# ScottHCL/recommend

Hardware: AMD Instinct MI355X
Metric: ranked samples/sec (fwd+bwd) at B=4096 seq=128; AUC parity vs ref (higher is better)
Workload: dtype f32-emulated (fp16-pair / split-bf16); 1 GPU; C2: OneTrans 4L d128 H4 f512 L_NS12 L_S128 (seq 3x42), Criteo-shape 13 dense + 26 ids, replicated tables, fwd+bwd+optimizer; global_batch=4096, per_gpu_batch=4096, seq_len=128, parallelism=dp1

## Files before the change

### include/onetrans_hip.h

```cpp
#ifndef ONETRANS_HIP_H
#define ONETRANS_HIP_H

#include <stddef.h>
#include <stdint.h>

#ifdef __cplusplus
extern "C" {
#endif

#define OT_OK 0
#define OT_ERR_INVALID_ARG 1
#define OT_ERR_UNSUPPORTED 2
#define OT_ERR_HIP 3

#define OT_GEMM_NN 0
#define OT_GEMM_NT 1

#define OT_AX_NONE 0
#define OT_AX_RMSNORM 1
#define OT_AX_GELU 2
#define OT_AX_BF16 4
#define OT_AX_BF16_RMSNORM 5

#define OT_EPI_BIAS 1
// ... 99 lines not shown
int ot_mixed_gemm_rms_img(int mode, const float* A, int64_t lda, int K, const int32_t* in_rows,
                          int a_xform, const float* a_rstd, const float* a_gamma,
                          const float* W, int64_t w_gstride, int64_t ldw, int N,
                          const int32_t* tile_group, int ntiles,
                          const float* bias, int64_t bias_gstride,
                          float* C, int64_t ldc, const int32_t* out_rows, int epi,
                          const float* res, int64_t ldres, int res_tok,
                          const float* aux, int64_t ldaux,
                          uint32_t seed, uint32_t site, float drop_rate, int tail_K, int tail_I,
                          const int32_t* tail_pos, const ot_rms_epilogue* rms, const uint16_t* b_image,
                          int image_ntn, int image_tn0, int precision, void* stream);

typedef struct ot_ffn_fused_args {
  size_t struct_size;
  const float* x1; int64_t ldx1;
  const int32_t* rows;
  const int32_t* tile_group; int ntiles;
  const float* rstd;
  const uint16_t* w1_image; int w1_groups;
  const uint16_t* w2_image; int w2_groups;
  const float* b1; int64_t b1_gstride;
  const float* b2; int64_t b2_gstride;
  int f;
  float* u_out; int64_t ldu;
  float* u_amax;
  float* x2; int64_t ldx2;
  float* rstd_out; float eps;
  uint32_t seed, site; float drop_rate;
  int tail_K, tail_I; const int32_t* tail_pos;
} ot_ffn_fused_args;
int ot_ffn_fused_fwd(const ot_ffn_fused_args* args, void* stream);
int ot_ffn_fused(int on);

int ot_attn_fwd(const float* qkv, int64_t ld, int B, int H, int I, int K, const int32_t* qpos,
                int head_dim, float* out, float* lse, int precision, void* stream);
size_t ot_attn_fwd_fp8_workspace_size(int B, int H, int I, int head_dim);
int ot_attn_fwd_fp8(const float* qkv, int64_t ld, int B, int H, int I, int K, const int32_t* qpos,
                    int head_dim, float* out, float* lse, void* workspace, size_t ws_bytes, void* stream);
#define OT_FP8_DEQUANT 1
#define OT_FP8_TWO_TERM 2
int ot_attn_fwd_fp8_ex(float* qkv, int64_t ld, int B, int H, int I, int K, const int32_t* qpos, int head_dim,
                       float* out, float* lse, void* workspace, size_t ws_bytes, int flags, void* stream);
int ot_attn_fwd_fp8_deq16(const float* qkv, int64_t ld, int B, int H, int I, int K, const int32_t* qpos,
                          int head_dim, float* out, float* lse, void* workspace, size_t ws_bytes, int flags,
                          uint16_t* deq16, void* stream);
size_t ot_attn_bwd_workspace_size(int B, int H, int K);
int ot_attn_bwd(const float* qkv, int64_t ld, const float* out, const float* dout, const float* lse,
                int B, int H, int I, int K, const int32_t* qpos, int head_dim, float* dqkv, float* delta_ws,
                int precision, void* stream);
size_t ot_attn_bwd_ex_workspace_size(int B, int H, int I, int K, int head_dim, int selected, int precision);
int ot_attn_bwd_ex(const float* qkv, int64_t ld, const float* out, const float* dout, const float* lse,
                   int B, int H, int I, int K, const int32_t* qpos, int head_dim, float* dqkv, void* workspace,
                   size_t ws_bytes, int precision, void* stream);
#define OT_ATTN_DQKV_BF16 1
#define OT_ATTN_QKV_BF16 2
#define OT_ATTN_DQ_PART_BF16 4
int ot_attn_bwd_dqkv_bf16_supported(int I, int K, int head_dim, int selected, int precision);
int ot_attn_bwd_bf16_forms(int I, int K, int head_dim, int selected, int precision);
size_t ot_attn_bwd_flags_workspace_size(int B, int H, int I, int K, int head_dim, int selected, int flags, int precision);
int ot_attn_slice_supported(int I, int K, int head_dim, int selected);
int ot_attn_bwd_flags(const float* qkv, int64_t ld, const float* out, const float* dout, const float* lse,
                      int B, int H, int I, int K, const int32_t* qpos, int head_dim, void* dqkv, int flags,
                      void* workspace, size_t ws_bytes, int precision, void* stream);
int ot_attn_amax_supported(int I, int K, int head_dim, int selected, int precision);
int ot_attn_fwd_amax(const float* qkv, int64_t ld, int B, int H, int I, int K, const int32_t* qpos,
                     int head_dim, float* out, float* lse, float* amax, float* rowmax, int precision, void* stream);
// ... 211 lines not shown
```

### recommend_amd/_lib.py

```python

from __future__ import annotations

import ctypes
import os
from ctypes import c_float, c_int, c_int64, c_size_t, c_uint32, c_void_p, c_char_p

_HERE = os.path.dirname(os.path.abspath(__file__))
LIB_PATH = os.environ.get('ONETRANS_HIP_LIB') or os.path.join(_HERE, 'libonetrans_hip.so')
HEADER = os.path.join(os.path.dirname(_HERE), 'include', 'onetrans_hip.h')

OT_GEMM_NN, OT_GEMM_NT = 0, 1
OT_AX_NONE, OT_AX_RMSNORM, OT_AX_GELU, OT_AX_BF16, OT_AX_BF16_RMSNORM = 0, 1, 2, 4, 5
OT_EPI_BIAS, OT_EPI_GELU_BWD, OT_EPI_GELU = 1, 2, 4
OT_EPI_DROPOUT, OT_EPI_RESIDUAL, OT_EPI_ACCUMULATE = 8, 16, 32
OT_EPI_ROW_RSTD, OT_EPI_RMSNORM_BWD, OT_EPI_ROWDOT = 64, 128, 256
OT_EPI_C_BF16 = 512
OT_EPI_AUX_BF16 = 1024
OT_ATTN_DQKV_BF16 = 1
OT_ATTN_QKV_BF16 = 2
OT_ATTN_DQ_PART_BF16 = 4
OT_WG_D_BF16 = 8
OT_MATMUL_F32, OT_MATMUL_SPLIT_BF16, OT_MATMUL_BF16 = 0, 1, 2
OT_FP8_DEQUANT, OT_FP8_TWO_TERM = 1, 2
OT_RANK_SUM, OT_RANK_PRODUCT = 0, 1
RANK_MODES = {'sum': OT_RANK_SUM, 'product': OT_RANK_PRODUCT}
RANK_MAX_K = 1024
MATMUL_MODES = {'f32': OT_MATMUL_F32, 'split': OT_MATMUL_SPLIT_BF16, 'bf16': OT_MATMUL_BF16}


class RmsEpilogue(ctypes.Structure):
    _fields_ = [('struct_size', c_size_t), ('rstd_out', c_void_p), ('eps', c_float),
                ('x', c_void_p), ('ldx', c_int64), ('gamma', c_void_p), ('rstd', c_void_p),
                ('dres', c_void_p), ('lddres', c_int64), ('dres_tail_K', c_int), ('dres_tail_I', c_int),
                ('dres_tail_inv', c_void_p),
                ('dx_masked', c_void_p), ('lddxm', c_int64),
                ('dgamma', c_void_p), ('accumulate_dgamma', c_int),
                ('workspace', c_void_p), ('ws_bytes', c_size_t),
                ('rowdot', c_void_p), ('rowdot_n', c_int),
                ('gelu_out', c_void_p), ('ldgelu', c_int64),
                ('xn_out', c_void_p), ('ldxn', c_int64),
                ('c16_out', c_void_p), ('ldc16', c_int64),
                ('rowmax_out', c_void_p), ('rowmax_n', c_int),
                ('a_rowmax', c_void_p), ('a_rowmax_n', c_int),
                ('amax_out', c_void_p), ('rowabs_out', c_void_p), ('rowabs_n', c_int)]

class FfnFusedArgs(ctypes.Structure):
    _fields_ = [('struct_size', c_size_t), ('x1', c_void_p), ('ldx1', c_int64), ('rows', c_void_p),
                ('tile_group', c_void_p), ('ntiles', c_int), ('rstd', c_void_p),
                ('w1_image', c_void_p), ('w1_groups', c_int), ('w2_image', c_void_p), ('w2_groups', c_int),
                ('b1', c_void_p), ('b1_gstride', c_int64), ('b2', c_void_p), ('b2_gstride', c_int64),
                ('f', c_int), ('u_out', c_void_p), ('ldu', c_int64), ('u_amax', c_void_p),
                ('x2', c_void_p), ('ldx2', c_int64), ('rstd_out', c_void_p), ('eps', c_float),
                ('seed', c_uint32), ('site', c_uint32), ('drop_rate', c_float),
                ('tail_K', c_int), ('tail_I', c_int), ('tail_pos', c_void_p)]


class SeqTime(ctypes.Structure):
    _fields_ = [('times', c_void_p), ('stride_b', c_int64), ('L', ctypes.c_int32), ('map_off', ctypes.c_int32)]


class NsBag(ctypes.Structure):
    _fields_ = [('table', c_void_p), ('ids', c_void_p), ('weights', c_void_p), ('row_offset', c_int64),
                ('num_rows', c_int64), ('ids_stride', c_int64), ('weights_stride', c_int64),
                ('width', ctypes.c_int32), ('cap', ctypes.c_int32), ('col', ctypes.c_int32),
                ('pooling', ctypes.c_int32)]


OT_BAG_SUM, OT_BAG_MEAN = 0, 1
BAG_POOLINGS = {'sum': OT_BAG_SUM, 'mean': OT_BAG_MEAN}
NS_BAG_MAX = 32
NS_BAG_MAX_WIDTH = 256
SEQ_TIME_MAX_L = 4096
SEQ_TIME_MAX_SEQ = 32

P = c_void_p
I64 = c_int64

SIGNATURES = {
    'ot_version': (c_int, []),
    'ot_get_last_error_string': (c_char_p, []),
    'ot_gemm_tile_rows': (c_int, []),
    'ot_mixed_gemm': (c_int, [c_int, P, I64, c_int, P, c_int, P, P, P, I64, I64, c_int, P, c_int, P, I64,
                              P, I64, P, c_int, P, I64, c_int, P, I64, c_uint32, c_uint32, c_float, c_int,
                              c_int, P, c_int, P]),
    'ot_mixed_gemm_rms_workspace_size': (c_size_t, [c_int, c_int]),
    'ot_mixed_gemm_rms': (c_int, [c_int, P, I64, c_int, P, c_int, P, P, P, I64, I64, c_int, P, c_int, P, I64,
                                  P, I64, P, c_int, P, I64, c_int, P, I64, c_uint32, c_uint32, c_float, c_int,
                                  c_int, P, P, c_int, P]),
    'ot_wgrad_workspace_size': (c_size_t, [c_int, c_int, c_int]),
    'ot_mixed_gemm_wgrad': (c_int, [P, I64, P, c_int, P, P, P, I64, P, c_int, c_int, P, c_int, P, c_int, P,
                                    I64, P, I64, c_int, P, c_size_t, c_int, P]),
    'ot_mixed_gemm_wgrad_ex': (c_int, [P, I64, P, c_int, P, P, P, I64, P, c_int, c_int, P, c_int, P, c_int, P,
                                       I64, P, I64, c_int, P, c_size_t, P, P, c_int, P]),
    'ot_transpose_banks': (c_int, [P, P, P, c_int, I64, P]),
    'ot_mixed_gemm_img': (c_int, [c_int, P, I64, c_int, P, c_int, P, P, P, I64, I64, c_int, P, c_int, P, I64,
                                  P, I64, P, c_int, P, I64, c_int, P, I64, c_uint32, c_uint32, c_float, c_int,
                                  c_int, P, P, c_int, c_int, c_int, P]),
    'ot_mixed_gemm_rms_img': (c_int, [c_int, P, I64, c_int, P, c_int, P, P, P, I64, I64, c_int, P, c_int, P, I64,
                                      P, I64, P, c_int, P, I64, c_int, P, I64, c_uint32, c_uint32, c_float, c_int,
                                      c_int, P, P, P, c_int, c_int, c_int, P]),
    'ot_split_image_elems': (c_size_t, [c_int, c_int, c_int]),
    'ot_plane_wide': (c_int, [c_int]),
    'ot_wgrad_wide': (c_int, [c_int]),
    'ot_plane_rowmeta': (c_int, [c_int]),
    'ot_plane_panel': (c_int, [c_int]),
    'ot_plane_panel_launches': (c_int, []),
    'ot_ffn_fused_fwd': (c_int, [P, P]),
    'ot_ffn_fused': (c_int, [c_int]),
    'ot_split_images': (c_int, [P, P, c_int, I64, P, c_int, P]),
    'ot_attn_fwd': (c_int, [P, I64, c_int, c_int, c_int, c_int, P, c_int, P, P, c_int, P]),
    'ot_attn_fwd_fp8_workspace_size': (c_size_t, [c_int, c_int, c_int, c_int]),
    'ot_attn_fwd_fp8': (c_int, [P, I64, c_int, c_int, c_int, c_int, P, c_int, P, P, P, c_size_t, P]),
    'ot_attn_fwd_fp8_ex': (c_int, [P, I64, c_int, c_int, c_int, c_int, P, c_int, P, P, P, c_size_t, c_int, P]),
    'ot_attn_fwd_fp8_deq16': (c_int, [P, I64, c_int, c_int, c_int, c_int, P, c_int, P, P, P, c_size_t, c_int, P, P]),
    'ot_attn_bwd_workspace_size': (c_size_t, [c_int, c_int, c_int]),
    'ot_attn_bwd': (c_int, [P, I64, P, P, P, c_int, c_int, c_int, c_int, P, c_int, P, P, c_int, P]),
    'ot_attn_bwd_ex_workspace_size': (c_size_t, [c_int, c_int, c_int, c_int, c_int, c_int, c_int]),
    'ot_attn_bwd_ex': (c_int, [P, I64, P, P, P, c_int, c_int, c_int, c_int, P, c_int, P, P, c_size_t, c_int, P]),
    'ot_attn_bwd_dqkv_bf16_supported': (c_int, [c_int, c_int, c_int, c_int, c_int]),
    'ot_attn_bwd_bf16_forms': (c_int, [c_int, c_int, c_int, c_int, c_int]),
    'ot_attn_slice_supported': (c_int, [c_int, c_int, c_int, c_int]),
    'ot_attn_bwd_flags_workspace_size': (c_size_t, [c_int, c_int, c_int, c_int, c_int, c_int, c_int, c_int]),
    'ot_attn_bwd_flags': (c_int, [P, I64, P, P, P, c_int, c_int, c_int, c_int, P, c_int, P, c_int, P, c_size_t, c_int, P]),
    'ot_attn_fwd_cached': (c_int, [P, I64, P, I64, P, c_int, c_int, c_int, c_int, c_int, c_int, P, P]),
    'ot_attn_fwd_cached_lse': (c_int, [P, I64, P, I64, P, c_int, c_int, c_int, c_int, c_int, c_int, P, P, P]),
    'ot_attn_bwd_cached_workspace_size': (c_size_t, [c_int, c_int, c_int, c_int, c_int, c_int, c_int]),
    'ot_attn_bwd_cached': (c_int, [P, I64, P, I64, P, c_int, c_int, c_int, c_int, c_int, c_int, c_int, P, P, P, P, P,
                                   c_int, P, c_size_t, P]),
    'ot_attn_amax_supported': (c_int, [c_int, c_int, c_int, c_int, c_int]),
    'ot_attn_fwd_amax': (c_int, [P, I64, c_int, c_int, c_int, c_int, P, c_int, P, P, P, P, c_int, P]),
    'ot_attn_bwd_amax': (c_int, [P, I64, P, P, P, c_int, c_int, c_int, c_int, P, c_int, P, P, c_size_t, P, P, c_int,
                                 P]),
    'ot_pyramid_select': (c_int, [P, c_float, c_int, c_int, c_int, c_int, P, P, P, c_int, P]),
    'ot_rmsnorm_fwd': (c_int, [P, I64, P, P, I64, P, I64, c_int, c_float, P]),
    'ot_rmsnorm_bwd_workspace_size': (c_size_t, [I64, c_int]),
    'ot_rmsnorm_bwd': (c_int, [P, I64, P, I64, P, P, P, I64, c_int, c_int, P, P, I64, P, I64, c_uint32,
                               c_uint32, c_float, c_int, c_int, P, P, c_int, I64, c_int, P, c_size_t, P]),
    'ot_dropout_apply': (c_int, [P, I64, P, I64, I64, c_int, c_uint32, c_uint32, c_float, c_int, c_int, P, P]),
    'ot_dropout_apply_bf16': (c_int, [P, I64, P, I64, I64, c_int, c_uint32, c_uint32, c_float, c_int, c_int, P, P]),
    'ot_rows_absmax': (c_int, [P, I64, I64, c_int, P, c_int, P]),
    'ot_dropout_rowmax_supported': (c_int, [c_int]),
# ... 115 lines not shown
```

### recommend_amd/csrc/gemm_ffn.hip

```cpp
#include <atomic>
#include <cstdlib>
#include <mutex>

#include "gemm.h"

namespace ot {

#ifndef OT_FFN_NSTG
#define OT_FFN_NSTG 3
#endif
constexpr int FF_NST = OT_FFN_NSTG;
static_assert(FF_NST == 2 || FF_NST == 3, "fused FFN stage buffers");
constexpr int PG_A_BYTES = GT * 16 * 4;
constexpr int FF_STG = PG_A_BYTES + 2 * GT * 16 * 2;
constexpr int FF_TR_LD = 36;
constexpr int FF_TR_WAVE = 32 * FF_TR_LD * 4;
constexpr int FF_TR_OFF = FF_NST * FF_STG;
constexpr int FF_META_OFF = FF_TR_OFF + 4 * FF_TR_WAVE;
constexpr int FF_TAB_OFF = FF_META_OFF + GT * 4;
constexpr int FF_MAX_F = 1024;
static_assert(FF_META_OFF >= (64 * (GT + 4) + 8 * GT) * 4, "fused FFN: the epilogue tile overlays the row metadata");
static_assert(FF_TAB_OFF + (2 * FF_MAX_F + GT) * 4 <= 80 * 1024, "fused FFN LDS");
constexpr int ffn_lds(int f) { return FF_TAB_OFF + (2 * f + GT) * 4; }

// ... 210 lines not shown
          }
#pragma unroll
        for (int nb = 0; nb < 4; ++nb) acc2[nb] = mfma_pair_t(fw[nb], fh, acc2[nb]);
      }
    };
    stage2(0, acc1[0]);
    stage2(1, acc1[1]);
    stage2(2, acc1[2]);
    stage2(3, acc1[3]);
  }
#pragma unroll
  for (int nb = 0; nb < 4; ++nb)
#pragma unroll
    for (int qd = 0; qd < 4; ++qd) {
      const f32x4 cs = *reinterpret_cast<const f32x4*>(tab + 2 * q.f + 32 * nb + 8 * qd + 4 * h);
#pragma unroll
      for (int i = 0; i < 4; ++i) acc2[nb][4 * qd + i] *= hinv * cs[i];
    }
  asm volatile("s_waitcnt vmcnt(0) lgkmcnt(0)" ::: "memory");
  __syncthreads();
  gemm_vec_epilogue<EPIT, 5, false, 8, false>(p, acc2, smem, tm, 0, g, 0, -1, rmeta);
  if (q.u_amax) amax_flush(q.u_amax, am);
}

#ifndef OT_FFN_FUSED
#define OT_FFN_FUSED 1
#endif
static int ffn_fused_initial() {
  const char* e = getenv("ONETRANS_FFN_FUSED");
  return e && *e ? (atoi(e) != 0) : OT_FFN_FUSED;
}
static std::atomic<int> g_ffn_fused{ffn_fused_initial()};

}

using namespace ot;

extern "C" int ot_ffn_fused(int on) {
  const int old = g_ffn_fused.load(std::memory_order_relaxed);
  if (on >= 0) g_ffn_fused.store(on ? 1 : 0, std::memory_order_relaxed);
  return old;
}

extern "C" int ot_ffn_fused_fwd(const ot_ffn_fused_args* a, void* stream) {
  OT_REQUIRE(a, "ot_ffn_fused_fwd: null arguments");
  OT_REQUIRE(a->struct_size == sizeof(ot_ffn_fused_args),
             "ot_ffn_fused_fwd: ot_ffn_fused_args.struct_size %zu != %zu (header of another ot_version)",
             a->struct_size, sizeof(ot_ffn_fused_args));
  OT_REQUIRE(a->x1 && a->x2 && a->rstd && a->w1_image && a->w2_image && a->b1 && a->b2,
             "ot_ffn_fused_fwd: null operand");
  OT_REQUIRE(a->ntiles >= 0 && a->f >= GT && a->f % GT == 0 && a->f <= FF_MAX_F,
             "ot_ffn_fused_fwd: bad sizes ntiles=%d f=%d (f a multiple of %d up to %d)", a->ntiles, a->f, GT, FF_MAX_F);
  auto a16 = [](const void* q) { return ((uintptr_t)q & 15) == 0; };
  OT_REQUIRE(a->ldx1 >= GT && a->ldx2 >= GT && a->ldx1 % 4 == 0 && a->ldx2 % 4 == 0 && a16(a->x1) && a16(a->x2) &&
                 a16(a->b1) && a16(a->b2) && a->b1_gstride % 4 == 0 && a->b2_gstride % 4 == 0 && a16(a->w1_image) &&
                 a16(a->w2_image),
             "ot_ffn_fused_fwd: rows of %d floats, leading dimensions and bias strides multiples of 4, 16-B aligned "
             "operands", GT);
  OT_REQUIRE(!a->u_out || (a->ldu >= a->f && a->ldu % 4 == 0 && a16(a->u_out)),
             "ot_ffn_fused_fwd: u_out needs ldu >= f, ldu %% 4 == 0 and 16-B alignment");
  OT_REQUIRE(a->w1_groups >= 1 && a->w2_groups >= 1, "ot_ffn_fused_fwd: image group counts must be >= 1");
  OT_REQUIRE(a->w1_groups == 1 && a->w2_groups == 1 ? true : a->tile_group != nullptr,
             "ot_ffn_fused_fwd: grouped weight images need tile_group");
  OT_REQUIRE(a->drop_rate >= 0.f && a->drop_rate < 1.f, "ot_ffn_fused_fwd: drop_rate out of range");
  OT_REQUIRE(a->drop_rate == 0.f || (a->tail_K > 0 && a->tail_I >= a->tail_K), "ot_ffn_fused_fwd: bad tail map");
  if (a->ntiles == 0) return OT_OK;
  FfnArgs q{};
  GemmArgs& p = q.e;
  p.A = a->x1; p.lda = a->ldx1; p.K = GT; p.in_rows = a->rows; p.a_xform = OT_AX_RMSNORM; p.a_rstd = a->rstd;
// ... 43 lines not shown
```

### recommend_amd/kernels.py

```python

from __future__ import annotations

import contextlib
import ctypes
import functools
import os
import threading
from typing import Optional, Tuple, Union

import torch

from . import _lib
from ._lib import call, size

Ptrish = Union[None, torch.Tensor, Tuple[torch.Tensor, int]]


class Probe:

    def __init__(self):
        self.recs = []

    def begin(self):
        ev = torch.cuda.Event(enable_timing=True)
# ... 277 lines not shown
    return _lib.size('ot_plane_panel', int(on))


def plane_panel_launches() -> int:
    return _lib.size('ot_plane_panel_launches')


def ffn_fused(on: int = -1) -> int:
    return _lib.size('ot_ffn_fused', int(on))


FFN_FUSED_MAX_F = 1024


def ffn_fused_fwd(x1: Ptrish, ldx1: int, rows: Ptrish, tile_group: Ptrish, ntiles: int, rstd: Ptrish, w1_image,
                  w1_groups: int, w2_image, w2_groups: int, b1: Ptrish, b1_gstride: int, b2: Ptrish, b2_gstride: int,
                  f: int, x2: Ptrish, ldx2: int, *, u_out: Ptrish = None, ldu: int = 0, u_amax: Ptrish = None,
                  rstd_out: Ptrish = None, eps: float = 1e-6, seed: int = 0, site: int = 0, drop: float = 0.0,
                  tail: Tuple[int, int] = (1, 1), m_rows: int = 0) -> None:
    a = _lib.FfnFusedArgs(ctypes.sizeof(_lib.FfnFusedArgs), ptr(x1), ldx1, ptr(rows), ptr(tile_group), ntiles,
                          ptr(rstd), ptr(w1_image), int(w1_groups), ptr(w2_image), int(w2_groups), ptr(b1),
                          b1_gstride, ptr(b2), b2_gstride, f, ptr(u_out), ldu, ptr(u_amax), ptr(x2), ldx2,
                          ptr(rstd_out), float(eps), seed & 0xFFFFFFFF, site, float(drop), tail[0], tail[1],
                          _sel(tail))
    ev = _probe.begin() if _probe is not None else None
    call('ot_ffn_fused_fwd', ctypes.byref(a), stream())
    if ev is not None:
        M = m_rows or ntiles * 128
        _probe.end('mixed_gemm', 2.0 * M * 128 * f * 2, ev, f'ffn_fused M{M} f{f} u{int(u_out is not None)}',
                   4.0 * M * 128 * 3 + 4.0 * M * f * (u_out is not None)
                   + 4.0 * M * (1 + (rstd_out is not None)), 3)


def split_images(base, desc_dev, ndesc, total_units, img) -> None:
    call('ot_split_images', ptr(base), ptr(desc_dev), ndesc, total_units, ptr(img), _prec(), stream())


def attn_fwd(qkv: torch.Tensor, ld: int, B: int, H: int, I: int, K: int, hd: int, out: torch.Tensor,
             lse: torch.Tensor, qpos: Optional[torch.Tensor] = None, fp8: bool = False,
             dequant: bool = False, fp8_terms: int = 1, deq16: Optional[torch.Tensor] = None,
             amax: Optional[torch.Tensor] = None, rowmax: Optional[torch.Tensor] = None) -> None:
    if fp8 and fp8_terms not in (1, 2):
        raise ValueError(f'fp8_terms {fp8_terms}: 1 or 2')
    ws = None
    if fp8:
        ws = workspace(size('ot_attn_fwd_fp8_workspace_size', B, H, I, hd), qkv.device)
    ev = _probe.begin() if _probe is not None else None
    if fp8 and deq16 is not None:
        call('ot_attn_fwd_fp8_deq16', ptr(qkv), ld, B, H, I, K, ptr(qpos), hd, ptr(out), ptr(lse), ptr(ws),
             ws.numel(), _lib.OT_FP8_TWO_TERM if fp8_terms == 2 else 0, ptr(deq16), stream())
    elif fp8:
        call('ot_attn_fwd_fp8_ex', ptr(qkv), ld, B, H, I, K, ptr(qpos), hd, ptr(out), ptr(lse), ptr(ws),
             ws.numel(), (_lib.OT_FP8_DEQUANT if dequant else 0) | (_lib.OT_FP8_TWO_TERM if fp8_terms == 2 else 0),
             stream())
    elif amax is not None or rowmax is not None:
        call('ot_attn_fwd_amax', ptr(qkv), ld, B, H, I, K, ptr(qpos), hd, ptr(out), ptr(lse), ptr(amax), ptr(rowmax),
             _prec(), stream())
    else:
        call('ot_attn_fwd', ptr(qkv), ld, B, H, I, K, ptr(qpos), hd, ptr(out), ptr(lse), _prec(), stream())
    if ev is not None:
        _probe.end('attention', 4.0 * (K * I - K * (K - 1) / 2) * hd * H * B, ev,
                   f'fwd{"_fp8" if fp8 else ""} I{I} K{K} hd{hd}')


def attn_bwd_bf16_forms(I, K, hd, qpos=None) -> int:
    return int(_lib.load().ot_attn_bwd_bf16_forms(I, K, hd, int(qpos is not None), _prec()))
# ... 477 lines not shown
```

### recommend_amd/model.py

```python

from __future__ import annotations

import json
import os
from typing import Dict, List, Optional, Tuple

import numpy as np
import torch
import torch.nn as nn

from . import _lib
from . import kernels as K
from ._lib import (OT_AX_BF16, OT_AX_BF16_RMSNORM, OT_AX_GELU, OT_AX_RMSNORM, OT_EPI_ACCUMULATE, OT_EPI_AUX_BF16, OT_EPI_BIAS,
                   OT_EPI_C_BF16, OT_EPI_DROPOUT, OT_EPI_GELU_BWD, OT_EPI_RESIDUAL, OT_EPI_RMSNORM_BWD,
                   OT_EPI_ROW_RSTD, OT_EPI_ROWDOT, OT_GEMM_NN, OT_GEMM_NT, OT_WG_D_BF16, NS_FIELD_BYTES)
from .config import (OneTransConfig, check_bag_features, check_padding_mask, check_pyramid_select, check_seq_fusion,
                     get_model_config)
from .layout import TILE, FlatLayout, RowMap, build_map, head_map, identity_map, layer_maps, round_up
from .params import init_params, ns_table_offsets

RMS_EPS = 1e-6


class _Tokenize(torch.autograd.Function):
# ... 369 lines not shown
        nca, nct = maps['all'].chunks.shape[0], maps['tail'].chunks.shape[0]
        G = cfg.num_groups
        dx2 = dx2.contiguous()
        rowdot = None
        fused2 = m.fuse_bwd2 and not m.fuse_bwd and f % TILE == 0
        du_bf = (fused2 and h is not None and m.bimg(f'blk.{l}.w1', 'dgrad') is not None)
        out = (lambda name: bounds.out(l, name)) if bounds is not None else (lambda name: None)
        b_o, b_u = (bounds.get(l, 'o'), bounds.get(l, 'u')) if bounds is not None else (None, None)
        keep = (bounds.t,) if bounds is not None else ()
        pw2, pw1, pwo = (m.dgrad_pair(f'blk.{l}.{w}') for w in ('w2', 'w1', 'wo'))
        dy2_rep = rate > 0 and not du_bf
        b_dy2 = out('dy2') if dy2_rep else None
        rm_dy2 = (torch.empty(B * Kq, (d + 255) // 256, device=dev)
                  if dy2_rep and pw2 and K.dropout_rowmax_supported(d) else None)
        dy2 = dx2
        if rate > 0:
            dy2 = torch.empty(B * Kq, d, device=dev, dtype=torch.int16 if du_bf else torch.float32)
            K.dropout_apply(dx2, d, dy2, d, B * Kq, d, seed, 2 * l + 1, rate, tail, amax=b_dy2, rowmax=rm_dy2)
        pa2 = a_row_bounds(pw2, dy2, d, B * Kq, d, rm_dy2)
        dy_bf = dy2.dtype == torch.int16
        du = torch.empty(B * Kq, f, device=dev, dtype=torch.int16 if du_bf else torch.float32)
        cbf = OT_EPI_C_BF16 if du_bf else 0
        hbf = (torch.empty(B * Kq, f, dtype=torch.int16, device=dev)
               if h is None and fused2 and K.matmul_mode() == 'bf16' else None)
        if hbf is None:
            with m.side(u if h is None else h, dy2, *keep):
                K.wgrad(u if h is None else h, f, mt['rows'][1], dy2, d, mt['rows'][1], f, d, mt, nct, G,
                        m.g(f'blk.{l}.w2'), f * d, m.g(f'blk.{l}.b2'), d,
                        a_xform=(OT_AX_GELU if h is None else OT_AX_BF16) | (OT_WG_D_BF16 if dy_bf else 0),
                        accumulate=acc, device=dev, m_rows=maps['tail'].nrows, rowmap=maps['tail'],
                        a_bound=b_u if h is None else None, d_bound=b_dy2)
        du_rep = fused2 or (((bounds is not None and not du_bf) or pw2 or pw1) and f % TILE == 0)
        b_du = out('du') if du_rep and not du_bf else None
        rm_du = torch.empty(B * Kq, f // TILE, device=dev) if pw1 and du_rep else None
        rep_du = dict(amax_out=b_du, rowabs_out=rm_du, rowabs_n=f // TILE if rm_du is not None else 0)
        if fused2:
            rowdot = torch.empty(B * Kq, f // TILE, device=dev)
            K.gemm_rms(OT_GEMM_NT, dy2, d, d, mt['rows'][1], m.p(f'blk.{l}.w2'), f * d, d, f, mt['tile_group'], nt,
                       du, f, mt['rows'][1], aux=u, ldaux=f, a_xform=OT_AX_BF16 if dy_bf else 0,
                       epi=OT_EPI_GELU_BWD | OT_EPI_ROWDOT | cbf | (OT_EPI_AUX_BF16 if u.dtype == torch.int16 else 0),
                       bias=m.p(f'blk.{l}.b1'), bias_gstride=f, rowdot=rowdot, rowdot_n=f // TILE,
                       m_rows=maps['tail'].nrows, device=dev, bimg=m.bimg(f'blk.{l}.w2', 'dgrad'),
                       gelu_out=hbf, ldgelu=f, **rep_du, **pa2)
            if hbf is not None:
                with m.side(hbf, dy2):
                    K.wgrad(hbf, f, mt['rows'][1], dy2, d, mt['rows'][1], f, d, mt, nct, G, m.g(f'blk.{l}.w2'),
                            f * d, m.g(f'blk.{l}.b2'), d, a_xform=OT_AX_BF16, accumulate=acc, device=dev,
                            m_rows=maps['tail'].nrows, rowmap=maps['tail'])
        else:
            K.gemm_rms(OT_GEMM_NT, dy2, d, d, mt['rows'][1], m.p(f'blk.{l}.w2'), f * d, d, f, mt['tile_group'], nt, du,
                       f, mt['rows'][1], epi=OT_EPI_GELU_BWD, aux=u, ldaux=f, m_rows=maps['tail'].nrows, device=dev,
                       bimg=m.bimg(f'blk.{l}.w2', 'dgrad'), **rep_du, **pa2)
        pa1 = a_row_bounds(pw1, du, f, B * Kq, f, rm_du)
        a1n = x1n is not None and du_bf
        with m.side(x1n if a1n else x1, du, rstd2, *keep):
            K.wgrad(x1n if a1n else x1, d, mt['rows'][1], du, f, mt['rows'][1], d, f, mt, nct, G, m.g(f'blk.{l}.w1'),
                    d * f, m.g(f'blk.{l}.b1'), f, rstd=rstd2, gamma=m.p(f'blk.{l}.norm2'),
                    a_xform=(OT_AX_BF16 if a1n else OT_AX_RMSNORM) | (OT_WG_D_BF16 if du_bf else 0),
                    accumulate=acc, device=dev, m_rows=maps['tail'].nrows, rowmap=maps['tail'], d_bound=b_du)
        dx1 = torch.empty(B * Kq, d, device=dev)
        dyo = torch.empty(B * Kq, d, device=dev) if rate > 0 else dx1
        dx1_ep = m.fuse_bwd or rowdot is not None
        rm_dyo = torch.empty(B * Kq, (d + TILE - 1) // TILE, device=dev) if pwo and dx1_ep else None
        b_dyo = out('dyo') if dx1_ep else None
        if dx1_ep:
            K.gemm_rms(OT_GEMM_NT, du, f, f, mt['rows'][1], m.p(f'blk.{l}.w1'), d * f, f, d, mt['tile_group'], nt,
                       dx1, d, mt['rows'][1], epi=OT_EPI_RMSNORM_BWD | (OT_EPI_DROPOUT if rate > 0 else 0),
                       a_xform=OT_AX_BF16 if du_bf else 0,
                       seed=seed, site=2 * l, drop=rate, tail=tail, m_rows=maps['tail'].nrows, nx=x1, ldnx=d,
                       ngamma=m.p(f'blk.{l}.norm2'), nrstd=rstd2, dres=dx2, lddres=d,
                       dx_masked=dyo if rate > 0 else None, lddxm=d, dgamma=m.g(f'blk.{l}.norm2'),
                       accumulate_dgamma=acc, device=dev, bimg=m.bimg(f'blk.{l}.w1', 'dgrad'),
                       rowdot=rowdot, rowdot_n=f // TILE if rowdot is not None else 0, amax_out=b_dyo,
                       rowabs_out=rm_dyo, rowabs_n=rm_dyo.shape[1] if rm_dyo is not None else 0, **pa1)
        else:
            dxn2 = torch.empty(B * Kq, d, device=dev)
            K.gemm_rms(OT_GEMM_NT, du, f, f, mt['rows'][1], m.p(f'blk.{l}.w1'), d * f, f, d, mt['tile_group'], nt,
                       dxn2, d, mt['rows'][1], epi=0, m_rows=maps['tail'].nrows, device=dev,
                       bimg=m.bimg(f'blk.{l}.w1', 'dgrad'), **pa1)
            K.rmsnorm_bwd(dxn2, d, x1, d, m.p(f'blk.{l}.norm2'), rstd2, dx1, d, B * Kq, d, dres=dx2, lddres=d,
                          dx_masked=dyo if rate > 0 else None, lddxm=d, seed=seed, site=2 * l, drop=rate,
                          tail=tail, dgamma=m.g(f'blk.{l}.norm2'), accumulate=acc, device=dev)
        with m.side(o, dyo, *keep):
            _wgrad_single(m, o, dyo, d, d, mt, m.g(f'blk.{l}.wo'), acc, dev, maps['tail'].nrows, maps['tail'],
                          a_bound=b_o, d_bound=b_dyo)
        do = torch.empty(B * Kq, d, device=dev)
        K.gemm_rms(OT_GEMM_NT, dyo, d, d, mt['rows'][1], m.p(f'blk.{l}.wo'), 0, d, d, mt['tile_group'], nt, do, d,
                   mt['rows'][1], epi=0, m_rows=maps['tail'].nrows, device=dev, bimg=m.bimg(f'blk.{l}.wo', 'dgrad'),
                   **a_row_bounds(pwo, dyo, d, B * Kq, d, rm_dyo))
        if yf is not None:
            dx = _fold_backward(m, l, x, rstd1, qkv, o, lse, yf, do, dx1, B, I, maps['fold'], acc, dev)
            m.side_block_done()
            if m.grad_ready is not None:
                m.grad_ready(l)
            return None, dx, None, None, None, None, None, None, None, None, None, None
        qp = _attn_qpos(cfg, pos)
        dq_bf = (K.matmul_mode() == 'bf16'
                 and K.attn_bwd_bf16_forms(I, Kq, hd, qp) & _lib.OT_ATTN_DQKV_BF16
# ... 881 lines not shown
```

Baseline: 211,000 samples/s.

## Fuse FFN backward dgrad GEMMs with GELU-grad and RMSNorm-bwd epilogue

Adds a fused kernel for the FFN backward pass. It computes du = (dy2·W2ᵀ)⊙gelu'(u) one 128-column chunk at a time and feeds each chunk straight into the dx1 = du·W1ᵀ accumulation, finishing with the RMSNorm-backward, dropout and dgamma epilogue. This removes the round trip of du through global memory as the A operand of the second GEMM, one kernel launch, and the per-row du rowabs pass. du is still written out for the weight-gradient GEMM. The cost is a running rescale of the pair-split accumulator as the bound grows across chunks, which could affect precision, and one block processes the whole f dimension serially.

Measured after the change: 213,400 samples/s (median of 6 runs). 1.01x the previous value.

```diff
diff --git a/include/onetrans_hip.h b/include/onetrans_hip.h
--- a/include/onetrans_hip.h
+++ b/include/onetrans_hip.h
@@ -155,6 +155,32 @@
 int ot_ffn_fused_fwd(const ot_ffn_fused_args* args, void* stream);
 int ot_ffn_fused(int on);
 
+typedef struct ot_ffn_fused_bwd_args {
+  size_t struct_size;
+  const float* dy2; int64_t lddy2;
+  const float* dy2_rowmax; int dy2_rowmax_n;
+  const int32_t* rows;
+  const int32_t* tile_group; int ntiles;
+  const uint16_t* w2_image; int w2_groups;
+  const uint16_t* w1_image; int w1_groups;
+  int f;
+  const float* u; int64_t ldu;
+  float* du; int64_t lddu;
+  float* du_amax;
+  const float* x1; int64_t ldx1;
+  const float* gamma; const float* rstd;
+  const float* dres; int64_t lddres;
+  float* dx1; int64_t lddx1;
+  float* dx_masked; int64_t lddxm;
+  float* dgamma; int accumulate_dgamma;
+  void* workspace; size_t ws_bytes;
+  float* amax_out; float* rowabs_out; int rowabs_n;
+  uint32_t seed, site; float drop_rate;
+  int tail_K, tail_I; const int32_t* tail_pos;
+} ot_ffn_fused_bwd_args;
+int ot_ffn_fused_bwd(const ot_ffn_fused_bwd_args* args, void* stream);
+int ot_ffn_fused_bwd_on(int on);
+
 int ot_attn_fwd(const float* qkv, int64_t ld, int B, int H, int I, int K, const int32_t* qpos,
                 int head_dim, float* out, float* lse, int precision, void* stream);
 size_t ot_attn_fwd_fp8_workspace_size(int B, int H, int I, int head_dim);
diff --git a/recommend_amd/_lib.py b/recommend_amd/_lib.py
--- a/recommend_amd/_lib.py
+++ b/recommend_amd/_lib.py
@@ -51,6 +51,21 @@
                 ('b1', c_void_p), ('b1_gstride', c_int64), ('b2', c_void_p), ('b2_gstride', c_int64),
                 ('f', c_int), ('u_out', c_void_p), ('ldu', c_int64), ('u_amax', c_void_p),
                 ('x2', c_void_p), ('ldx2', c_int64), ('rstd_out', c_void_p), ('eps', c_float),
+                ('seed', c_uint32), ('site', c_uint32), ('drop_rate', c_float),
+                ('tail_K', c_int), ('tail_I', c_int), ('tail_pos', c_void_p)]
+
+
+class FfnFusedBwdArgs(ctypes.Structure):
+    _fields_ = [('struct_size', c_size_t), ('dy2', c_void_p), ('lddy2', c_int64),
+                ('dy2_rowmax', c_void_p), ('dy2_rowmax_n', c_int), ('rows', c_void_p),
+                ('tile_group', c_void_p), ('ntiles', c_int),
+                ('w2_image', c_void_p), ('w2_groups', c_int), ('w1_image', c_void_p), ('w1_groups', c_int),
+                ('f', c_int), ('u', c_void_p), ('ldu', c_int64), ('du', c_void_p), ('lddu', c_int64),
+                ('du_amax', c_void_p), ('x1', c_void_p), ('ldx1', c_int64), ('gamma', c_void_p), ('rstd', c_void_p),
+                ('dres', c_void_p), ('lddres', c_int64), ('dx1', c_void_p), ('lddx1', c_int64),
+                ('dx_masked', c_void_p), ('lddxm', c_int64), ('dgamma', c_void_p), ('accumulate_dgamma', c_int),
+                ('workspace', c_void_p), ('ws_bytes', c_size_t),
+                ('amax_out', c_void_p), ('rowabs_out', c_void_p), ('rowabs_n', c_int),
                 ('seed', c_uint32), ('site', c_uint32), ('drop_rate', c_float),
                 ('tail_K', c_int), ('tail_I', c_int), ('tail_pos', c_void_p)]
 
@@ -107,6 +122,8 @@
     'ot_plane_panel_launches': (c_int, []),
     'ot_ffn_fused_fwd': (c_int, [P, P]),
     'ot_ffn_fused': (c_int, [c_int]),
+    'ot_ffn_fused_bwd': (c_int, [P, P]),
+    'ot_ffn_fused_bwd_on': (c_int, [c_int]),
     'ot_split_images': (c_int, [P, P, c_int, I64, P, c_int, P]),
     'ot_attn_fwd': (c_int, [P, I64, c_int, c_int, c_int, c_int, P, c_int, P, P, c_int, P]),
     'ot_attn_fwd_fp8_workspace_size': (c_size_t, [c_int, c_int, c_int, c_int]),
diff --git a/recommend_amd/csrc/gemm_ffn.hip b/recommend_amd/csrc/gemm_ffn.hip
--- a/recommend_amd/csrc/gemm_ffn.hip
+++ b/recommend_amd/csrc/gemm_ffn.hip
@@ -266,9 +266,342 @@
 }
 static std::atomic<int> g_ffn_fused{ffn_fused_initial()};
 
+constexpr int FB_TAB_OFF = FF_TAB_OFF;
+static_assert(FB_TAB_OFF + (FF_MAX_F + GT) * 4 <= 80 * 1024, "fused FFN backward LDS");
+constexpr int ffn_bwd_lds(int f) { return FB_TAB_OFF + (f + GT) * 4; }
+
+struct FfnBwdArgs {
+  GemmArgs e;
+  const uint16_t* img2; int g2;
+  const uint16_t* img1; int g1;
+  const float* u; int64_t ldu;
+  float* du; int64_t lddu;
+  float* du_amax;
+  int f;
+};
+
+template <int EPIT>
+__global__ __launch_bounds__(256, 2) void ffn_fused_bwd_kernel(FfnBwdArgs q) {
+  const GemmArgs& p = q.e;
+  extern __shared__ __attribute__((aligned(16))) float smem[];
+  char* lds = reinterpret_cast<char*>(smem);
+  const int tm = xcd_remap(blockIdx.x, p.ntm);
+  const int g = p.tile_group ? p.tile_group[tm] : 0;
+  const int t = threadIdx.x, lane = t & 63, wave = t >> 6;
+  const int h = lane >> 5, li = lane & 31;
+  const int nch = q.f >> 7;
+
+  int arow[2];
+#pragma unroll
+  for (int i = 0; i < 2; ++i) {
+    const int64_t gr = (int64_t)tm * GT + (2 * wave + i) * 16 + (lane >> 2);
+    const int ir = p.in_rows ? p.in_rows[gr] : (int)gr;
+    arow[i] = ir < 0 ? 0 : ir;
+  }
+  int urow[4];
+#pragma unroll
+  for (int i = 0; i < 4; ++i) {
+    const int64_t gr = (int64_t)tm * GT + 32 * wave + 8 * i + (lane >> 3);
+    const int ur = p.out_rows ? p.out_rows[gr] : (int)gr;
+    urow[i] = ur < 0 ? 0 : ur;
+  }
+  constexpr int64_t T1 = 8 * (int64_t)PG_B_BYTES;
+  const char* img2 = reinterpret_cast<const char*>(q.img2) + (int64_t)(q.g2 ? g : 0) * nch * T1;
+  const char* img1 = reinterpret_cast<const char*>(q.img1) + (int64_t)(q.g1 ? g : 0) * (q.f >> 4) * PG_B_BYTES;
+  const int blane = 2 * wave * 1024 + 16 * lane;
+  auto issue = [&](int c, int sidx, int buf) {
+    char* sb = lds + buf * FF_STG;
+    if (sidx < 8) {
+      const char* bs = img2 + c * T1 + (int64_t)sidx * PG_B_BYTES + blane;
+#pragma unroll
+      for (int i = 0; i < 2; ++i)
+        __builtin_amdgcn_global_load_lds(
+            (const void*)(p.A + (int64_t)arow[i] * p.lda + 16 * sidx + 4 * ((lane & 3) ^ ((lane >> 4) & 3))),
+            (lds_void_t*)(sb + (2 * wave + i) * 1024), 16, 0, 0);
+#pragma unroll
+      for (int i = 0; i < 2; ++i)
+        __builtin_amdgcn_global_load_lds((const void*)(bs + i * 1024),
+                                         (lds_void_t*)(sb + PG_A_BYTES + (2 * wave + i) * 1024), 16, 0, 0);
+    } else if (sidx < 12) {
+#pragma unroll
+      for (int i = 0; i < 4; ++i)
+        __builtin_amdgcn_global_load_lds(
+            (const void*)(q.u + (int64_t)urow[i] * q.ldu + 128 * c + 32 * (sidx - 8) +
+                          4 * ((lane & 7) ^ ((4 * i + (lane >> 4)) & 7))),
+            (lds_void_t*)(sb + (4 * wave + i) * 1024), 16, 0, 0);
+    } else {
+      const char* bs = img1 + (int64_t)(8 * c + 2 * (sidx - 12)) * PG_B_BYTES + blane;
+#pragma unroll
+      for (int u = 0; u < 2; ++u)
+#pragma unroll
+        for (int i = 0; i < 2; ++i)
+          __builtin_amdgcn_global_load_lds((const void*)(bs + u * PG_B_BYTES + i * 1024),
+                                           (lds_void_t*)(sb + u * 8192 + (2 * wave + i) * 1024), 16, 0, 0);
+    }
+  };
+
+  const int ra = 32 * wave + li;
+  const int aoff0 = ra * 64 + 16 * ((2 * h) ^ ((li >> 2) & 3));
+  const int sw = (li >> 3) & 1;
+  const int boff = PG_A_BYTES + li * 32 + 16 * (h ^ sw);
+  const int woff0 = li * 32 + 16 * sw + 8 * h;
+  const int usw = (li >> 1) & 7;
+
+  float abound = 0.f;
+  int mrow;
+  {
+    const int64_t gr = (int64_t)tm * GT + ra;
+    int ir = p.in_rows ? p.in_rows[gr] : (int)gr;
+    mrow = p.out_rows ? p.out_rows[gr] : (int)gr;
+    ir = ir < 0 ? 0 : ir;
+    for (int j = 0; j < p.a_rowmax_n; ++j) abound = fmaxf(abound, p.a_rowmax[(int64_t)ir * p.a_rowmax_n + j]);
+  }
+  float* tab = reinterpret_cast<float*>(lds + FB_TAB_OFF);
+  int tt = t;
+  asm volatile("" : "+v"(tt));
+  for (int idx = tt; idx < q.f; idx += 256) {
+    const float* cs = reinterpret_cast<const float*>(img2 + (idx >> 7) * T1 + 2 * GT * 16 * 2);
+    const float bad = reinterpret_cast<const uint32_t*>(cs)[GT] == PAIR_IMAGE_TAG ? 1.f : __builtin_nanf("");
+    tab[idx] = bad / cs[idx & 127];
+  }
+  if (tt < GT) {
+    const float* cs = reinterpret_cast<const float*>(img1 + 2 * GT * 16 * 2);
+    const float bad = reinterpret_cast<const uint32_t*>(cs)[GT] == PAIR_IMAGE_TAG ? 1.f : __builtin_nanf("");
+    tab[q.f + tt] = bad / cs[tt];
+  }
+  int* rmeta = reinterpret_cast<int*>(lds + FF_META_OFF);
+  if (h == 0) rmeta[ra] = mrow;
+  const float asc = pow2_scale14(abound);
+  const float ainv = 1.f / asc;
+  float* trw = reinterpret_cast<float*>(lds + FF_TR_OFF + wave * FF_TR_WAVE);
+  asm volatile("" : "+v"(abound), "+v"(mrow), "+v"(arow[0]), "+v"(arow[1]), "+v"(urow[0]), "+v"(urow[1]),
+               "+v"(urow[2]), "+v"(urow[3]));
+
+  int rb = 0;
+  issue(0, 0, 0);
+  if (FF_NST == 3) issue(0, 1, 1);
+  f32x16 acc2[4];
+#pragma unroll
+  for (int a = 0; a < 4; ++a)
+#pragma unroll
+    for (int r = 0; r < 16; ++r) acc2[a][r] = 0.f;
+  float am = 0.f, bound = 0.f, hsc = 1.f, hinv = 1.f;
+
+  for (int c = 0; c < nch; ++c) {
+    auto top = [&](int sidx) -> const char* {
+      if (FF_NST == 2 || sidx == 12 || (sidx == 15 && c + 1 == nch)) asm volatile("s_waitcnt vmcnt(0)" ::: "memory");
+      else asm volatile("s_waitcnt vmcnt(4)" ::: "memory");
+      asm volatile("s_waitcnt lgkmcnt(0)" ::: "memory");
+      __builtin_amdgcn_s_barrier();
+      asm volatile("" ::: "memory");
+      constexpr int AH = FF_NST - 1;
+      const int nb_ = rb == 0 ? FF_NST - 1 : rb - 1;
+      if (sidx + AH < 16) issue(c, sidx + AH, nb_);
+      else if (c + 1 < nch) issue(c + 1, sidx + AH - 16, nb_);
+      const char* sb = lds + rb * FF_STG;
+      rb = rb + 1 == FF_NST ? 0 : rb + 1;
+      return sb;
+    };
+    f32x16 acc1[4];
+#pragma unroll
+    for (int a = 0; a < 4; ++a)
+#pragma unroll
+      for (int r = 0; r < 16; ++r) acc1[a][r] = 0.f;
+#pragma unroll
+    for (int kt = 0; kt < 8; ++kt) {
+      const char* sb = top(kt);
+      u32x4 fb[4][2];
+#pragma unroll
+      for (int nb = 0; nb < 4; ++nb)
+#pragma unroll
+        for (int pl = 0; pl < 2; ++pl) fb[nb][pl] = *reinterpret_cast<const u32x4*>(sb + boff + pl * 4096 + nb * 1024);
+      const f32x4 a0 = *reinterpret_cast<const f32x4*>(sb + aoff0);
+      const f32x4 a1 = *reinterpret_cast<const f32x4*>(sb + (aoff0 ^ 16));
+      const float av[8] = {a0.x, a0.y, a0.z, a0.w, a1.x, a1.y, a1.z, a1.w};
+      u32x4 fa[3];
+      pair8(av, asc, fa);
+#pragma unroll
+      for (int nb = 0; nb < 4; ++nb) acc1[nb] = mfma_pair_t(fb[nb], fa, acc1[nb]);
+    }
+    float ua = 0.f;
+    auto finish = [&](int nb, f32x16& a) {
+      const char* sb = top(8 + nb);
+#pragma unroll
+      for (int qd = 0; qd < 4; ++qd) {
+        const f32x4 u4 = *reinterpret_cast<const f32x4*>(sb + ra * 128 + 16 * ((2 * qd + h) ^ usw));
+        const f32x4 ci = *reinterpret_cast<const f32x4*>(tab + 128 * c + 32 * nb + 8 * qd + 4 * h);
+        f32x4 v = {a[4 * qd], a[4 * qd + 1], a[4 * qd + 2], a[4 * qd + 3]};
+        v = v * (ainv * ci);
+        v *= gelu_erf_grad4(u4);
+        ua = amax4(ua, v);
+        a[4 * qd] = v.x; a[4 * qd + 1] = v.y; a[4 * qd + 2] = v.z; a[4 * qd + 3] = v.w;
+      }
+    };
+    finish(0, acc1[0]);
+    finish(1, acc1[1]);
+    finish(2, acc1[2]);
+    finish(3, acc1[3]);
+    if (mrow >= 0) am = fmaxf(am, ua);
+    bound = fmaxf(bound, fmaxf(ua, __shfl_xor(ua, 32, 64)));
+    {
+      const float s = pow2_scale14(bound);
+      if (c > 0) {
+        const float ratio = s * hinv;
+#pragma unroll
+        for (int a = 0; a < 4; ++a)
+#pragma unroll
+          for (int r = 0; r < 16; ++r) acc2[a][r] *= ratio;
+      }
+      hsc = s;
+      hinv = 1.f / s;
+    }
+#pragma unroll
+    for (int nb = 0; nb < 4; ++nb) {
+#pragma unroll
+      for (int qd = 0; qd < 4; ++qd)
+        *reinterpret_cast<f32x4*>(trw + li * FF_TR_LD + 8 * qd + 4 * h) =
+            f32x4{acc1[nb][4 * qd], acc1[nb][4 * qd + 1], acc1[nb][4 * qd + 2], acc1[nb][4 * qd + 3]};
+      asm volatile("s_waitcnt lgkmcnt(0)" ::: "memory");
+#pragma unroll
+      for (int ps = 0; ps < 4; ++ps) {
+        const f32x4 v = *reinterpret_cast<const f32x4*>(trw + ((lane >> 3) + 8 * ps) * FF_TR_LD + 4 * (lane & 7));
+        const int ur = rmeta[32 * wave + (lane >> 3) + 8 * ps];
+        if (ur >= 0) store_out4(q.du + (int64_t)ur * q.lddu + 128 * c + 32 * nb + 4 * (lane & 7), v);
+      }
+      asm volatile("s_waitcnt lgkmcnt(0)" ::: "memory");
+    }
+    auto stage2 = [&](int j, const f32x16& u) {
+      const char* sb = top(12 + j);
+#pragma unroll
+      for (int s = 0; s < 2; ++s) {
+        const float hv[8] = {u[8 * s], u[8 * s + 1], u[8 * s + 2], u[8 * s + 3],
+                             u[8 * s + 4], u[8 * s + 5], u[8 * s + 6], u[8 * s + 7]};
+        u32x4 fh[3];
+        pair8(hv, hsc, fh);
+        u32x4 fw[4][2];
+#pragma unroll
+        for (int nb = 0; nb < 4; ++nb)
+#pragma unroll
+          for (int pl = 0; pl < 2; ++pl) {
+            const char* wb = sb + s * 8192 + pl * 4096 + nb * 1024;
+            const u32x2 lo = *reinterpret_cast<const u32x2*>(wb + woff0);
+            const u32x2 hi = *reinterpret_cast<const u32x2*>(wb + (woff0 ^ 16));
+            fw[nb][pl] = u32x4{lo.x, lo.y, hi.x, hi.y};
+          }
+#pragma unroll
+        for (int nb = 0; nb < 4; ++nb) acc2[nb] = mfma_pair_t(fw[nb], fh, acc2[nb]);
+      }
+    };
+    stage2(0, acc1[0]);
+    stage2(1, acc1[1]);
+    stage2(2, acc1[2]);
+    stage2(3, acc1[3]);
+  }
+#pragma unroll
+  for (int nb = 0; nb < 4; ++nb)
+#pragma unroll
+    for (int qd = 0; qd < 4; ++qd) {
+      const f32x4 cs = *reinterpret_cast<const f32x4*>(tab + q.f + 32 * nb + 8 * qd + 4 * h);
+#pragma unroll
+      for (int i = 0; i < 4; ++i) acc2[nb][4 * qd + i] *= hinv * cs[i];
+    }
+  asm volatile("s_waitcnt vmcnt(0) lgkmcnt(0)" ::: "memory");
+  __syncthreads();
+  gemm_vec_epilogue<EPIT, 5, false, OT_PLANE_EPI_RBN, false>(p, acc2, smem, tm, 0, g, 0, -1, rmeta);
+  if (q.du_amax) amax_flush(q.du_amax, am);
+}
+
+#ifndef OT_FFN_FUSED_BWD
+#define OT_FFN_FUSED_BWD 1
+#endif
+static int ffn_fused_bwd_initial() {
+  const char* e = getenv("ONETRANS_FFN_FUSED_BWD");
+  return e && *e ? (atoi(e) != 0) : OT_FFN_FUSED_BWD;
+}
+static std::atomic<int> g_ffn_fused_bwd{ffn_fused_bwd_initial()};
+
 }
 
 using namespace ot;
+
+extern "C" int ot_ffn_fused_bwd_on(int on) {
+  const int old = g_ffn_fused_bwd.load(std::memory_order_relaxed);
+  if (on >= 0) g_ffn_fused_bwd.store(on ? 1 : 0, std::memory_order_relaxed);
+  return old;
+}
+
+extern "C" int ot_ffn_fused_bwd(const ot_ffn_fused_bwd_args* a, void* stream) {
+  OT_REQUIRE(a, "ot_ffn_fused_bwd: null arguments");
+  OT_REQUIRE(a->struct_size == sizeof(ot_ffn_fused_bwd_args),
+             "ot_ffn_fused_bwd: ot_ffn_fused_bwd_args.struct_size %zu != %zu (header of another ot_version)",
+             a->struct_size, sizeof(ot_ffn_fused_bwd_args));
+  OT_REQUIRE(a->dy2 && a->dy2_rowmax && a->u && a->du && a->w2_image && a->w1_image && a->x1 && a->gamma && a->rstd &&
+                 a->dx1 && a->dgamma && a->workspace,
+             "ot_ffn_fused_bwd: null operand");
+  OT_REQUIRE(a->ntiles >= 0 && a->f >= GT && a->f % GT == 0 && a->f <= FF_MAX_F,
+             "ot_ffn_fused_bwd: bad sizes ntiles=%d f=%d (f a multiple of %d up to %d)", a->ntiles, a->f, GT, FF_MAX_F);
+  auto a16 = [](const void* q) { return ((uintptr_t)q & 15) == 0; };
+  OT_REQUIRE(a->lddy2 >= GT && a->ldx1 >= GT && a->lddx1 >= GT && a->lddy2 % 4 == 0 && a->ldx1 % 4 == 0 &&
+                 a->lddx1 % 4 == 0 && a16(a->dy2) && a16(a->x1) && a16(a->dx1) && a16(a->gamma) && a16(a->w2_image) &&
+                 a16(a->w1_image),
+             "ot_ffn_fused_bwd: rows of %d floats, leading dimensions multiples of 4, 16-B aligned operands", GT);
+  OT_REQUIRE(a->ldu >= a->f && a->lddu >= a->f && a->ldu % 4 == 0 && a->lddu % 4 == 0 && a16(a->u) && a16(a->du),
+             "ot_ffn_fused_bwd: u / du need ld >= f, ld %% 4 == 0 and 16-B alignment");
+  OT_REQUIRE(a->dy2_rowmax_n >= 1, "ot_ffn_fused_bwd: dy2_rowmax_n must be >= 1");
+  OT_REQUIRE(!a->dres || (a->lddres >= GT && a->lddres % 4 == 0 && a16(a->dres)),
+             "ot_ffn_fused_bwd: dres needs lddres >= %d, lddres %% 4 == 0 and 16-B alignment", GT);
+  OT_REQUIRE(a->w1_groups >= 1 && a->w2_groups >= 1, "ot_ffn_fused_bwd: image group counts must be >= 1");
+  OT_REQUIRE(a->w1_groups == 1 && a->w2_groups == 1 ? true : a->tile_group != nullptr,
+             "ot_ffn_fused_bwd: grouped weight images need tile_group");
+  OT_REQUIRE(a->drop_rate >= 0.f && a->drop_rate < 1.f, "ot_ffn_fused_bwd: drop_rate out of range");
+  OT_REQUIRE(a->drop_rate == 0.f || (a->tail_K > 0 && a->tail_I >= a->tail_K), "ot_ffn_fused_bwd: bad tail map");
+  OT_REQUIRE(a->drop_rate == 0.f || (a->dx_masked && a->lddxm >= GT && a->lddxm % 4 == 0 && a16(a->dx_masked)),
+             "ot_ffn_fused_bwd: dropout needs dx_masked (lddxm >= %d, lddxm %% 4 == 0, 16-B aligned)", GT);
+  OT_REQUIRE(a->ws_bytes >= ot_mixed_gemm_rms_workspace_size(a->ntiles, GT), "ot_ffn_fused_bwd: workspace too small");
+  OT_REQUIRE(!a->rowabs_out || a->rowabs_n == 1, "ot_ffn_fused_bwd: rowabs_out needs rowabs_n == 1");
+  if (a->ntiles == 0) return OT_OK;
+  FfnBwdArgs q{};
+  GemmArgs& p = q.e;
+  p.A = a->dy2; p.lda = a->lddy2; p.K = a->f; p.in_rows = a->rows;
+  p.a_rowmax = a->dy2_rowmax; p.a_rowmax_n = a->dy2_rowmax_n;
+  p.N = GT; p.tile_group = a->tile_group;
+  p.C = a->dx1; p.ldc = a->lddx1; p.out_rows = a->rows;
+  p.seed = a->seed; p.site = a->site; p.drop_thr = 0u; p.drop_scale = 1.f;
+  p.tail_K = a->tail_K > 0 ? a->tail_K : 1; p.tail_I = a->tail_I > 0 ? a->tail_I : 1; p.tail_pos = a->tail_pos;
+  p.drop_width = GT; p.ntm = a->ntiles; p.ntn = 1;
+  p.nx = a->x1; p.ldnx = a->ldx1; p.ngamma = a->gamma; p.nrstd = a->rstd;
+  p.dres = a->dres; p.lddres = a->lddres;
+  p.dxm = a->dx_masked; p.lddxm = a->lddxm;
+  p.dgpart = (float*)a->workspace;
+  p.amax_out = a->amax_out; p.rowabs_out = a->rowabs_out; p.rowabs_n = a->rowabs_n;
+  int epi = OT_EPI_RMSNORM_BWD;
+  if (a->drop_rate > 0.f) {
+    epi |= OT_EPI_DROPOUT;
+    p.drop_thr = drop_threshold(a->drop_rate);
+    p.drop_scale = 1.f / (1.f - a->drop_rate);
+  }
+  p.epi = epi;
+  q.img2 = a->w2_image; q.g2 = a->w2_groups > 1;
+  q.img1 = a->w1_image; q.g1 = a->w1_groups > 1;
+  q.u = a->u; q.ldu = a->ldu; q.du = a->du; q.lddu = a->lddu; q.du_amax = a->du_amax; q.f = a->f;
+  void (*kern)(FfnBwdArgs) = a->drop_rate > 0.f ? ffn_fused_bwd_kernel<OT_EPI_RMSNORM_BWD | OT_EPI_DROPOUT>
+                                                : ffn_fused_bwd_kernel<OT_EPI_RMSNORM_BWD>;
+  static std::once_flag once;
+  std::call_once(once, [] {
+    (void)hipFuncSetAttribute((const void*)ffn_fused_bwd_kernel<OT_EPI_RMSNORM_BWD>,
+                              hipFuncAttributeMaxDynamicSharedMemorySize, ffn_bwd_lds(FF_MAX_F));
+    (void)hipFuncSetAttribute((const void*)ffn_fused_bwd_kernel<OT_EPI_RMSNORM_BWD | OT_EPI_DROPOUT>,
+                              hipFuncAttributeMaxDynamicSharedMemorySize, ffn_bwd_lds(FF_MAX_F));
+    (void)hipGetLastError();
+  });
+  hipStream_t s = (hipStream_t)stream;
+  hipLaunchKernelGGL(kern, dim3((unsigned)a->ntiles), dim3(256), (size_t)ffn_bwd_lds(a->f), s, q);
+  OT_LAUNCH_CHECK("ot_ffn_fused_bwd");
+  float* dgpart = (float*)a->workspace;
+  launch_colsum_reduce(dgpart, a->ntiles, GT, a->dgamma, a->accumulate_dgamma, s, dgpart + (int64_t)a->ntiles * GT);
+  OT_LAUNCH_CHECK("ot_ffn_fused_bwd(dgamma)");
+  return OT_OK;
+}
 
 extern "C" int ot_ffn_fused(int on) {
   const int old = g_ffn_fused.load(std::memory_order_relaxed);
diff --git a/recommend_amd/kernels.py b/recommend_amd/kernels.py
--- a/recommend_amd/kernels.py
+++ b/recommend_amd/kernels.py
@@ -333,6 +333,34 @@
                    + 4.0 * M * (1 + (rstd_out is not None)), 3)
 
 
+def ffn_fused_bwd_on(on: int = -1) -> int:
+    return _lib.size('ot_ffn_fused_bwd_on', int(on))
+
+
+def ffn_fused_bwd(dy2: Ptrish, lddy2: int, dy2_rowmax: Ptrish, dy2_rowmax_n: int, rows: Ptrish, tile_group: Ptrish,
+                  ntiles: int, w2_image, w2_groups: int, w1_image, w1_groups: int, f: int, u: Ptrish, ldu: int,
+                  du: Ptrish, lddu: int, x1: Ptrish, ldx1: int, gamma: Ptrish, rstd: Ptrish, dx1: Ptrish, lddx1: int,
+                  dgamma: Ptrish, *, du_amax: Ptrish = None, dres: Ptrish = None, lddres: int = 0,
+                  dx_masked: Ptrish = None, lddxm: int = 0, accumulate_dgamma: bool = False, amax_out: Ptrish = None,
+                  rowabs_out: Ptrish = None, rowabs_n: int = 0, seed: int = 0, site: int = 0, drop: float = 0.0,
+                  tail: Tuple[int, int] = (1, 1), m_rows: int = 0, device=None) -> None:
+    ws = workspace(size('ot_mixed_gemm_rms_workspace_size', ntiles, 128),
+                   device if device is not None else (dx1[0] if isinstance(dx1, tuple) else dx1).device)
+    a = _lib.FfnFusedBwdArgs(ctypes.sizeof(_lib.FfnFusedBwdArgs), ptr(dy2), lddy2, ptr(dy2_rowmax), int(dy2_rowmax_n),
+                             ptr(rows), ptr(tile_group), ntiles, ptr(w2_image), int(w2_groups), ptr(w1_image),
+                             int(w1_groups), f, ptr(u), ldu, ptr(du), lddu, ptr(du_amax), ptr(x1), ldx1, ptr(gamma),
+                             ptr(rstd), ptr(dres), lddres, ptr(dx1), lddx1, ptr(dx_masked), lddxm, ptr(dgamma),
+                             int(accumulate_dgamma), ptr(ws), ws.numel(), ptr(amax_out), ptr(rowabs_out),
+                             int(rowabs_n), seed & 0xFFFFFFFF, site, float(drop), tail[0], tail[1], _sel(tail))
+    ev = _probe.begin() if _probe is not None else None
+    call('ot_ffn_fused_bwd', ctypes.byref(a), stream())
+    if ev is not None:
+        M = m_rows or ntiles * 128
+        _probe.end('mixed_gemm', 2.0 * M * 128 * f * 2, ev, f'ffn_fused_bwd M{M} f{f} drop{int(drop > 0)}',
+                   4.0 * M * 128 * (3 + (dres is not None) + (dx_masked is not None)) + 4.0 * M * f * 2
+                   + 4.0 * M * (1 + dy2_rowmax_n), 3)
+
+
 def split_images(base, desc_dev, ndesc, total_units, img) -> None:
     call('ot_split_images', ptr(base), ptr(desc_dev), ndesc, total_units, ptr(img), _prec(), stream())
 
diff --git a/recommend_amd/model.py b/recommend_amd/model.py
--- a/recommend_amd/model.py
+++ b/recommend_amd/model.py
@@ -425,9 +425,24 @@
                         a_bound=b_u if h is None else None, d_bound=b_dy2)
         du_rep = fused2 or (((bounds is not None and not du_bf) or pw2 or pw1) and f % TILE == 0)
         b_du = out('du') if du_rep and not du_bf else None
-        rm_du = torch.empty(B * Kq, f // TILE, device=dev) if pw1 and du_rep else None
+        ffn_bwd = (pw2 and pw1 and m.fuse_bwd and d == TILE and f % TILE == 0 and f <= K.FFN_FUSED_MAX_F
+                   and not du_bf and h is None and bool(K.ffn_fused_bwd_on()))
+        rm_du = torch.empty(B * Kq, f // TILE, device=dev) if pw1 and du_rep and not ffn_bwd else None
         rep_du = dict(amax_out=b_du, rowabs_out=rm_du, rowabs_n=f // TILE if rm_du is not None else 0)
-        if fused2:
+        if ffn_bwd:
+            dx1 = torch.empty(B * Kq, d, device=dev)
+            dyo = torch.empty(B * Kq, d, device=dev) if rate > 0 else dx1
+            rm_dyo = torch.empty(B * Kq, 1, device=dev) if pwo else None
+            b_dyo = out('dyo')
+            K.ffn_fused_bwd(dy2, d, pa2['a_rowmax'], pa2['a_rowmax_n'], mt['rows'][1], mt['tile_group'], nt,
+                            m.bimg(f'blk.{l}.w2', 'dgrad')[0], m.layout.images[(f'blk.{l}.w2', 'dgrad')][1],
+                            m.bimg(f'blk.{l}.w1', 'dgrad')[0], m.layout.images[(f'blk.{l}.w1', 'dgrad')][1], f,
+                            u, f, du, f, x1, d, m.p(f'blk.{l}.norm2'), rstd2, dx1, d, m.g(f'blk.{l}.norm2'),
+                            du_amax=b_du, dres=dx2, lddres=d, dx_masked=dyo if rate > 0 else None, lddxm=d,
+                            accumulate_dgamma=acc, amax_out=b_dyo, rowabs_out=rm_dyo,
+                            rowabs_n=1 if rm_dyo is not None else 0, seed=seed, site=2 * l, drop=rate, tail=tail,
+                            m_rows=maps['tail'].nrows, device=dev)
+        elif fused2:
             rowdot = torch.empty(B * Kq, f // TILE, device=dev)
             K.gemm_rms(OT_GEMM_NT, dy2, d, d, mt['rows'][1], m.p(f'blk.{l}.w2'), f * d, d, f, mt['tile_group'], nt,
                        du, f, mt['rows'][1], aux=u, ldaux=f, a_xform=OT_AX_BF16 if dy_bf else 0,
@@ -444,19 +459,22 @@
             K.gemm_rms(OT_GEMM_NT, dy2, d, d, mt['rows'][1], m.p(f'blk.{l}.w2'), f * d, d, f, mt['tile_group'], nt, du,
                        f, mt['rows'][1], epi=OT_EPI_GELU_BWD, aux=u, ldaux=f, m_rows=maps['tail'].nrows, device=dev,
                        bimg=m.bimg(f'blk.{l}.w2', 'dgrad'), **rep_du, **pa2)
-        pa1 = a_row_bounds(pw1, du, f, B * Kq, f, rm_du)
+        pa1 = a_row_bounds(pw1, du, f, B * Kq, f, rm_du) if not ffn_bwd else {}
         a1n = x1n is not None and du_bf
         with m.side(x1n if a1n else x1, du, rstd2, *keep):
             K.wgrad(x1n if a1n else x1, d, mt['rows'][1], du, f, mt['rows'][1], d, f, mt, nct, G, m.g(f'blk.{l}.w1'),
                     d * f, m.g(f'blk.{l}.b1'), f, rstd=rstd2, gamma=m.p(f'blk.{l}.norm2'),
                     a_xform=(OT_AX_BF16 if a1n else OT_AX_RMSNORM) | (OT_WG_D_BF16 if du_bf else 0),
                     accumulate=acc, device=dev, m_rows=maps['tail'].nrows, rowmap=maps['tail'], d_bound=b_du)
-        dx1 = torch.empty(B * Kq, d, device=dev)
-        dyo = torch.empty(B * Kq, d, device=dev) if rate > 0 else dx1
         dx1_ep = m.fuse_bwd or rowdot is not None
-        rm_dyo = torch.empty(B * Kq, (d + TILE - 1) // TILE, device=dev) if pwo and dx1_ep else None
-        b_dyo = out('dyo') if dx1_ep else None
-        if dx1_ep:
+        if not ffn_bwd:
+            dx1 = torch.empty(B * Kq, d, device=dev)
+            dyo = torch.empty(B * Kq, d, device=dev) if rate > 0 else dx1
+            rm_dyo = torch.empty(B * Kq, (d + TILE - 1) // TILE, device=dev) if pwo and dx1_ep else None
+            b_dyo = out('dyo') if dx1_ep else None
+        if ffn_bwd:
+            pass
+        elif dx1_ep:
             K.gemm_rms(OT_GEMM_NT, du, f, f, mt['rows'][1], m.p(f'blk.{l}.w1'), d * f, f, d, mt['tile_group'], nt,
                        dx1, d, mt['rows'][1], epi=OT_EPI_RMSNORM_BWD | (OT_EPI_DROPOUT if rate > 0 else 0),
                        a_xform=OT_AX_BF16 if du_bf else 0,
```
